# slp-rl/aero

Hardware: AMD Instinct MI355X
Metric: real-time-factor (audio-sec/wall-sec), Aero.forward STFT+U-Net+iSTFT, 4->16kHz nfft=512 hop=64 batch=64 per GPU (higher is better)
Workload: dtype f16; 1 GPU; batch=64 synthetic 2s white-noise clips per GPU, 4->16 kHz, aero_4-16_512_64 (nfft=512 hop=64), random-init weights seed 2036, inference, inputs resident in HBM; global_batch=64, clip_samples=8000, frames=501, parallelism=clips sharded over 1 GPU(s), no data-path collective, precision=fp16 operands/storage, fp32 accumulate; STFT/iSTFT/statistics fp32

## Files before the change

### aero_amd/_lib.py

```python
import ctypes as C
import os

_HERE = os.path.dirname(os.path.abspath(__file__))
DEFAULT_LIB = os.path.join(_HERE, 'libaero_hip.so')

ACT_NONE, ACT_RELU, ACT_GELU, ACT_GLU, ACT_SNAKE = 0, 1, 2, 3, 4

i32, i64, vp, fp, dp = C.c_int32, C.c_int64, C.c_void_p, C.c_void_p, C.c_void_p


class ConvDesc(C.Structure):
    _fields_ = [('src0', vp), ('s0_b', i64), ('s0_f', i64), ('s0_t', i64), ('C0', i32),
                ('src1', vp), ('s1_b', i64), ('s1_f', i64), ('s1_t', i64), ('C1', i32),
                ('weight', vp), ('bias', fp),
                ('dst', vp), ('d_b', i64), ('d_f', i64), ('d_t', i64),
                ('dst_f32', i32), ('dst_f_off', i32), ('dst_F', i32),
                ('B', i32), ('Fin', i32), ('Fout', i32), ('T', i32), ('M', i32),
                ('transposed', i32), ('fstride', i32),
                ('ntaps', i32), ('df', i32 * 9), ('dt', i32 * 9),
                ('act', i32),
                ('res', vp), ('r_b', i64), ('r_f', i64), ('r_t', i64),
                ('post_add', fp), ('batch_scale', fp), ('batch_shift', fp),
                ('stats', dp), ('stat_count', C.c_double),
                ('stat_mode', i32), ('stat_G', i32), ('stat_per_row', i32), ('stat_eps', C.c_float),
# ... 103 lines not shown

class SeanetConvDesc(C.Structure):
    _fields_ = [('x', vp), ('wimg', vp), ('bias', fp), ('add', vp), ('y', vp),
                ('B', i32), ('Tin', i32), ('Cin', i32), ('Tq', i32), ('M', i32), ('K', i32), ('stride', i32), ('dil', i32), ('pad', i32),
                ('reflect', i32), ('ksteps', i32), ('R', i32), ('P', i32), ('Tout', i32), ('Cout', i32), ('act', i32), ('in_slope', C.c_float)]


class SeanetResDesc(C.Structure):
    _fields_ = [('x', vp), ('w1', vp), ('w2s', vp), ('b1', fp), ('b2s', fp), ('add', vp), ('y', vp),
                ('B', i32), ('T', i32), ('C', i32), ('d', i32), ('ks1', i32), ('ks2', i32), ('slope', C.c_float)]


DCONV_MAX_DEPTH = 4


class DconvLayer(C.Structure):
    _fields_ = [('w1', vp), ('w2', vp), ('consts', fp), ('snake_a', fp),
                ('dilation', i32), ('norm1', i32), ('norm2', i32), ('reserved', i32)]


class DconvDesc(C.Structure):
    _fields_ = [('x', vp), ('y', vp), ('R', i32), ('T', i32), ('C', i32), ('hidden', i32), ('depth', i32), ('act', i32),
                ('F', i32), ('eps', C.c_float), ('layer', DconvLayer * DCONV_MAX_DEPTH)]


_PROTOS = {
    'aero_version': (C.c_char_p, []),
    'aero_last_error': (C.c_char_p, []),
    'aero_last_kernel_name': (C.c_char_p, []),
    'aero_stft_fwd': (i32, [fp, i32, i32, i32, i32, i32, fp, i32, fp, i32, dp, i32, vp]),
    'aero_stft_dft_table_bytes': (i64, [i32]),
    'aero_stft_dft_table': (i32, [fp, i32, i32, vp, vp]),
    'aero_stft_dft_fwd': (i32, [fp, i32, i32, i32, i32, i32, i32, vp, fp, i32, dp, i32, vp]),
    'aero_stft_dft_norm_fwd': (i32, [fp, i32, i32, i32, i32, i32, i32, vp, i32, dp, i32, vp, fp, vp]),
    'aero_spec_normalize': (i32, [fp, i32, i64, dp, vp, fp, vp]),
    'aero_istft_fwd': (i32, [fp, i32, i32, i32, i32, i32, fp, fp, fp, i32, vp]),
    'aero_istft_pitch': (i32, [i32, i32, i32, C.POINTER(i32), C.POINTER(i32)]),
    'aero_istft_pitched_fwd': (i32, [fp, i32, i32, i32, i32, i32, i32, i32, fp, fp, fp, i32, vp]),
    'aero_conv_fwd': (i32, [C.POINTER(ConvDesc), vp]),
    'aero_split_finish': (i32, [fp, i32, fp, i32, vp, i64, i32, vp]),
    'aero_adam_step': (i32, [fp, fp, fp, fp, i64, C.c_float, C.c_float, C.c_float, C.c_float, i32, C.c_float, vp]),
    'aero_adam_step_dev': (i32, [fp, fp, fp, fp, i64, C.c_float, C.c_float, C.c_float, C.c_float, fp, C.c_float, vp]),
    'aero_conv_wgrad': (i32, [C.POINTER(WgradDesc), vp]),
    'aero_conv_wgrad_chunks': (i32, [i32, i32, i32, i32, i32]),
    'aero_norm_bwd_reduce': (i32, [C.POINTER(NormBwdDesc), vp]),
    'aero_norm_bwd_apply': (i32, [C.POINTER(NormBwdDesc), vp]),
    'aero_istft_bwd_prep': (i32, [fp, fp, fp, i32, i32, i32, i32, i32, vp]),
    'aero_istft_bwd_pack': (i32, [fp, fp, i32, i32, i32, i32, i32, vp]),
    'aero_conv_tile_m': (i32, [i32]),
    'aero_conv_ring_bm': (i32, [i32, i32]),
    'aero_convtr_tail_finish': (i32, [fp, fp, fp, fp, fp, fp, i32, i32, i32, i32, i32, vp]),
    'aero_convtr_tail_finish_pitched': (i32, [fp, fp, fp, fp, fp, fp, i32, i32, i32, i32, i32, i32, i32, vp]),
    'aero_conv_kernel_name': (i32, [C.POINTER(ConvDesc), C.c_char_p, i32]),
    'aero_norm_stats': (i32, [C.POINTER(NormDesc), vp]),
    'aero_norm_apply': (i32, [C.POINTER(NormDesc), vp]),
    'aero_gram_stats': (i32, [C.POINTER(GramDesc), vp]),
    'aero_lstm_fwd': (i32, [C.POINTER(LstmDesc), vp]),
    'aero_lstm_geometry': (i32, [i32, C.POINTER(i32), C.POINTER(i32)]),
    'aero_lstm_geometry_in': (i32, [i32, i32, C.POINTER(i32)]),
    'aero_localstate_fwd': (i32, [C.POINTER(AttnDesc), vp]),
    'aero_freqfc_fwd': (i32, [C.POINTER(FreqFcDesc), vp]),
    'aero_ftb_first_fwd': (i32, [C.POINTER(FtbFirstDesc), vp]),
    'aero_enc0_fwd': (i32, [C.POINTER(Enc0Desc), vp]),
    'aero_dconv_row_fwd': (i32, [C.POINTER(DconvDesc), vp]),
    'aero_dconv_row_fits': (i32, [i32, i32, i32, i32]),
    'aero_lstm_bwd': (i32, [C.POINTER(LstmBwdDesc), vp]),
    'aero_lstm_bwd_k4p': (i32, [i32]),
    'aero_localstate_bwd': (i32, [C.POINTER(AttnBwdDesc), vp]),
    'aero_freqfc_wgrad': (i32, [vp, vp, vp, fp, fp, i32, i32, i32, i32, i32, vp]),
    'aero_ftb_gate_bwd': (i32, [vp, vp, vp, vp, vp, vp, i32, i32, i32, i32, vp]),
    'aero_sum_bt': (i32, [vp, fp, i32, i32, i32, i32, C.c_float, vp]),
    'aero_frames_op': (i32, [vp, vp, i32, i32, i32, i32, i32, i32, i32, vp]),
    'aero_stft_loss_sums': (i32, [fp, fp, i64, C.c_float, dp, i32, dp, vp]),
    'aero_stft_loss_bwd': (i32, [fp, fp, i64, C.c_float, dp, C.c_float, C.c_float, fp, fp, vp]),
    'aero_irfft_frames': (i32, [fp, i32, i32, i32, i32, fp, fp, vp]),
    'aero_stft_adj_fold': (i32, [fp, fp, i32, i32, i32, i32, i32, i32, vp]),
    'aero_add_f16': (i32, [vp, vp, vp, i64, C.c_float, vp]),
    'aero_scale_cast': (i32, [fp, i32, i64, fp, vp, C.c_float, vp, fp, vp]),
    'aero_scale_f32': (i32, [fp, i64, fp, vp]),
    'aero_gather_pack': (i32, [vp, vp, i32, vp, vp, i64, i32, vp]),
    'aero_debug_probe': (i32, [vp, i32, i32, i32, vp, vp]),
    'aero_bn_running_update': (i32, [dp, i32, C.c_double, C.c_float, fp, fp, vp, vp]),
    'aero_gconv1d_mfma_ok': (i32, [i32, i32, i32, i32, i32, i32, i32]),
    'aero_weightnorm_fwd': (i32, [fp, fp, fp, i32, i32, vp]),
    'aero_weightnorm_bwd': (i32, [fp, i64, i64, i64, fp, fp, fp, fp, fp, fp, fp, fp, i32, i32, i32, i32, vp]),
    'aero_gconv1d_wgrad_slabs': (i32, [i32, i32, i32, i32, i32, i32, i32, i32, i32]),
    'aero_rescale_f16': (i32, [vp, fp, vp, fp, i64, vp, C.c_float, vp, fp, vp]),
    'aero_gconv1d_fwd': (i32, [C.POINTER(GconvDesc), vp]),
# ... 87 lines not shown
```

### aero_amd/csrc/aero_hip.hip

```cpp
#include "aero_common.h"
#ifdef AERO_PART
#define AERO_IN(p) (AERO_PART == (p))
#else
#define AERO_IN(p) 1
#endif
#if AERO_IN(0)
#include "k_attn.h"
#include "k_lstm.h"
#include "k_norm.h"
#include "k_gram.h"
#include "k_optim.h"
#endif
#if AERO_IN(1)
#include "k_stft.h"
#include "k_train.h"
#endif
#if AERO_IN(2)
#include "k_conv.h"
#endif
#if AERO_IN(6)
#include "k_conv_ring.h"
#endif
#if AERO_IN(7)
#include "k_pw.h"
// ... 399 lines not shown
    name[0] = 0;
    int rc = aero_conv_launch(d, nullptr, &err, name);
    return rc == AERO_OK ? AERO_OK : aero_fail(rc, err);
}

int aero_split_finish(const float* acc, int32_t nsplit, const float* bias, int32_t act, void* dst, int64_t npos, int32_t M, void* stream) {
    const char* err = "";
    int rc = aero_split_finish_launch(acc, nsplit, bias, act, dst, npos, M, (hipStream_t)stream, &err);
    return aero_finish(rc, err);
}

#endif

#if AERO_IN(3)

int aero_freqfc_fwd(const aero_freqfc_desc* d, void* stream) {
    const char* err = "";
    int rc = aero_freqfc_launch(d, (hipStream_t)stream, &err);
    return aero_finish(rc, err);
}

int aero_dconv_row_fwd(const aero_dconv_desc* d, void* stream) {
    const char* err = "";
    int rc = aero_dconv_launch(d, (hipStream_t)stream, &err);
    return aero_finish(rc, err);
}

int aero_dconv_row_fits(int T, int C, int hidden, int max_dilation) { return aero_dconv_row_fits_impl(T, C, hidden, max_dilation); }

int aero_enc0_fwd(const aero_enc0_desc* d, void* stream) {
    const char* err = "";
    int rc = aero_enc0_launch(d, (hipStream_t)stream, &err);
    return aero_finish(rc, err);
}

int aero_ftb_first_fwd(const aero_ftb_first_desc* d, void* stream) {
    const char* err = "";
    int rc = aero_ftb_first_launch(d, (hipStream_t)stream, &err);
    return aero_finish(rc, err);
}

#endif

#if AERO_IN(4)

int aero_conv_wgrad(const aero_wgrad_desc* d, void* stream) {
    const char* err = "";
    int rc = aero_conv_wgrad_launch(d, (hipStream_t)stream, &err);
    return aero_finish(rc, err);
}

// ... 342 lines not shown
```

### aero_amd/csrc/k_dconv.h

```cpp
#pragma once
#include "aero_common.h"

struct AeroDconvK {
    aero_dconv_desc d;
    int HP;
    int logp;
    int T16;
    int PADR;
};

static inline int aero_dconv_logp(int C) {
    int s = (2 * C) & 255, g = 256;
    if (s) g = s & -s;
    int P = 256 / g, l = 0;
    while ((1 << l) < P) ++l;
    return l;
}

static inline size_t aero_dconv_lds_bytes(int T, int C, int hidden, int maxdil) {
    if (T < 1 || C < 8 || C % 8 || hidden < 4 || hidden % 4 || hidden > 32 || maxdil < 1 || maxdil > 64) return 0;
    const int HP = (hidden + 15) / 16 * 16, K1p = (3 * C + 31) / 32 * 32, T16 = (T + 15) / 16 * 16;
    const int padr = (maxdil + 7) / 8 * 8;
    const int xrows = T16 + 2 * padr, logp = aero_dconv_logp(C);
    const size_t xs = (size_t)xrows * C + (size_t)((xrows >> logp) + 1) * 8;
    const size_t w1 = (size_t)HP * K1p, w2 = (size_t)2 * C * HP;
    const size_t halves = (xs + w1 + w2 + 7) / 8 * 8;
    const size_t floats = 3 * HP + 3 * 2 * C + C + 2 * 16 * 2 + 8;
    return halves * 2 + floats * 4;
}

static __device__ __forceinline__ void aero_dconv_moments(float s1, float s2, float inv_n, float eps, float& mean, float& rstd) {
    const float m = s1 * inv_n;
    double var = (double)s2 * (double)inv_n - (double)m * (double)m;
    const float vf = fmaxf((float)var, 0.f) + eps;
    float r = aero_rsqrt(vf);
    r = r * (1.5f - 0.5f * vf * r * r);
    mean = m;
    rstd = r;
}

static inline int aero_dconv_nw(size_t lds_bytes, int T) { return (lds_bytes > 80 * 1024 || T > 512) ? 16 : 8; }

template <int HM, int NF2, int NW, int MAXF>
__global__ __launch_bounds__(NW * 64, 4) void aero_dconv_row_kernel(AeroDconvK p) {
    constexpr int C = NF2 * 8, HP = HM * 16, NK1 = (3 * C + 31) / 32, K1p = NK1 * 32, CU = NF2, NT = NW * 64;
    const aero_dconv_desc& d = p.d;
    const int T = d.T, hidden = d.hidden;
    const int xrows = p.T16 + 2 * p.PADR;
    h16* xs = (h16*)AERO_DYN_SMEM;
    h16* w1s = xs + xrows * C + ((xrows >> p.logp) + 1) * 8;
    h16* w2s = w1s + HP * K1p;
    float* c1 = (float*)(xs + ((int)(w2s + 2 * C * HP - xs) + 7) / 8 * 8);
    float* c2 = c1 + 3 * HP;
    float* sc = c2 + 3 * 2 * C;
    float* red = sc + C;
    const int tid = threadIdx.x, lane = tid & 63, wave = aero_uniform(tid >> 6);
    const int g = lane >> 4, col = lane & 15;
    const int row = aero_xcd_swizzle((int)blockIdx.x, (int)gridDim.x);
    const int nfrag = p.T16 >> 4;
    auto xoff = [&](int r) { return r * C + ((r >> p.logp) << 3); };

    {
        const h16* src = (const h16*)d.x + (int64_t)row * T * C;
        const int gsz = (CU << p.logp) + 1;
        const int total = xrows * CU + (xrows >> p.logp) + 1;
        for (int ub = wave * 64; ub < total; ub += NT) {
// ... 155 lines not shown
        for (int mf = 0; mf < NF2; ++mf) {
            const f32x4 A2 = *(const f32x4*)&c2[2 * C + mf * 16 + g * 4], B2 = *(const f32x4*)&c2[4 * C + mf * 16 + g * 4];
            const f32x2 ls = *(const f32x2*)&sc[mf * 8 + g * 2];
            h16x4 wf[HM];
#pragma unroll
            for (int ks = 0; ks < HM; ++ks) wf[ks] = *(const h16x4*)&w2s[(mf * HM + ks) * 256 + w2lane];
#pragma unroll
            for (int f = 0; f < MAXF; ++f) {
                if (wave + f * NW >= nfrag) continue;
                h16* xr = &xs[xlane[f] + mf * 8];
                const h16x2 xv = *(const h16x2*)xr;
                f32x4 v = (f32x4){0.f, 0.f, 0.f, 0.f};
#pragma unroll
                for (int ks = 0; ks < HM; ++ks) v = __builtin_amdgcn_mfma_f32_16x16x16f16(wf[ks], hB[f][ks], v, 0, 0, 0);
                v = v * A2 + B2;
                constexpr float NL2E = -1.4426950408889634f;
                const float g0 = aero_rcp(1.f + aero_exp2(v[1] * NL2E)), g1 = aero_rcp(1.f + aero_exp2(v[3] * NL2E));
                const float o0 = fmaf(v[0] * g0, ls[0], (float)xv[0]);
                const float o1 = fmaf(v[2] * g1, ls[1], (float)xv[1]);
                if (msk[f] != 0.f) *(h16x2*)xr = (h16x2){(h16)o0, (h16)o1};
            }
        }
    }
    __syncthreads();
    {
        h16* dst = (h16*)d.y + (int64_t)row * T * C;
        for (int u = tid; u < T * CU; u += NT) {
            const int t = u / CU, s = u - t * CU;
            *(h16x8*)(dst + (int64_t)t * C + s * 8) = *(const h16x8*)&xs[xoff(t + p.PADR) + s * 8];
        }
    }
}

static int aero_dconv_row_fits_impl(int T, int C, int hidden, int maxdil) {
    const size_t b = aero_dconv_lds_bytes(T, C, hidden, maxdil);
    const int nf2 = C / 8;
    const bool inst = nf2 == 2 || nf2 == 4 || nf2 == 6 || nf2 == 8 || nf2 == 12 || nf2 == 16;
    return b != 0 && b <= 160 * 1024 && inst && T <= (nf2 >= 12 && aero_dconv_nw(b, T) == 16 ? 512 : 1024);
}

static int aero_dconv_launch(const aero_dconv_desc* d, hipStream_t stream, const char** err) {
    if (!d || !d->x || !d->y) { *err = "dconv: null pointer"; return AERO_ERR_ARG; }
    if (d->R < 1 || d->T < 1 || d->depth < 1 || d->depth > AERO_DCONV_MAX_DEPTH || d->F < 1) { *err = "dconv: bad geometry"; return AERO_ERR_ARG; }
    if (d->act != AERO_ACT_RELU && d->act != AERO_ACT_GELU && d->act != AERO_ACT_SNAKE && d->act != AERO_ACT_NONE) { *err = "dconv: unsupported act"; return AERO_ERR_UNSUPPORTED; }
    int maxdil = 1;
    for (int l = 0; l < d->depth; ++l) {
        const aero_dconv_layer& L = d->layer[l];
        if (!L.w1 || !L.w2 || !L.consts) { *err = "dconv: null layer weights"; return AERO_ERR_ARG; }
        if (d->act == AERO_ACT_SNAKE && !L.snake_a) { *err = "dconv: snake needs a"; return AERO_ERR_ARG; }
        if (L.dilation < 1) { *err = "dconv: dilation"; return AERO_ERR_ARG; }
        if ((((uintptr_t)L.w1 | (uintptr_t)L.w2 | (uintptr_t)L.consts) & 15)) { *err = "dconv: unaligned weights"; return AERO_ERR_ARG; }
        maxdil = L.dilation > maxdil ? L.dilation : maxdil;
    }
    if ((((uintptr_t)d->x | (uintptr_t)d->y) & 15)) { *err = "dconv: unaligned rows"; return AERO_ERR_ARG; }
    if (!aero_dconv_row_fits_impl(d->T, d->C, d->hidden, maxdil)) { *err = "dconv: row does not fit the LDS (or C % 8, hidden % 4, hidden > 32)"; return AERO_ERR_UNSUPPORTED; }
    if (d->R > 0x7fffffff) { *err = "dconv: grid too large"; return AERO_ERR_ARG; }
    AeroDconvK p;
    p.d = *d;
    p.HP = (d->hidden + 15) / 16 * 16;
    p.logp = aero_dconv_logp(d->C);
    p.T16 = (d->T + 15) / 16 * 16;
    p.PADR = (maxdil + 7) / 8 * 8;
    const size_t lds = aero_dconv_lds_bytes(d->T, d->C, d->hidden, maxdil);
    const int nw = aero_dconv_nw(lds, d->T), nf2 = d->C / 8;
    dim3 grid((unsigned)d->R), block((unsigned)nw * 64);
#define AERO_DCONV_GO(NF2_)                                                                                            \
    do {                                                                                                               \
        constexpr int MF16 = NF2_ >= 12 ? 2 : 4;      \
        if (nw == 16 && (d->T + 15) / 16 > 16 * MF16) { *err = "dconv: row too long"; return AERO_ERR_UNSUPPORTED; }    \
        if (p.HP == 16 && nw == 8) AERO_LAUNCH_DYN((aero_dconv_row_kernel<1, NF2_, 8, 4>), grid, block, lds, stream, p);  \
        else if (p.HP == 16) AERO_LAUNCH_DYN((aero_dconv_row_kernel<1, NF2_, 16, MF16>), grid, block, lds, stream, p);       \
        else if (nw == 8) AERO_LAUNCH_DYN((aero_dconv_row_kernel<2, NF2_, 8, 4>), grid, block, lds, stream, p);           \
        else AERO_LAUNCH_DYN((aero_dconv_row_kernel<2, NF2_, 16, MF16>), grid, block, lds, stream, p);                       \
    } while (0)
    switch (nf2) {
        case 2: AERO_DCONV_GO(2); break;
        case 4: AERO_DCONV_GO(4); break;
        case 6: AERO_DCONV_GO(6); break;
        case 8: AERO_DCONV_GO(8); break;
        case 12: AERO_DCONV_GO(12); break;
        default: AERO_DCONV_GO(16); break;
    }
#undef AERO_DCONV_GO
    return AERO_OK;
}
```

### aero_amd/engine.py

```python
import ctypes as C
import math
import os

import torch

from . import _lib, pack
from ._lib import ACT_GELU, ACT_GLU, ACT_NONE, ACT_RELU, ACT_SNAKE


def _ptr(t):
    return None if t is None else t.data_ptr()


def _strides4(t):
    assert t.dim() == 4 and (t.shape[3] == 1 or t.stride(3) == 1), (t.shape, t.stride())
    return t.stride(0), t.stride(1), t.stride(2)


_SIDE_STREAMS = {}


def side_streams(device, n):
    dev = torch.device(device)
    if dev.type == 'cuda' and dev.index is None:
# ... 209 lines not shown
        if split_acc is not None:
            self._call('aero_split_finish', 'aero_split_finish_kernel', 0.0, split_acc.numel() * 4 + dst.numel() * 2, _ptr(split_acc), tap_split,
                       _ptr(spec.bias), act, _ptr(dst), B * Fout * T, spec.M, self.stream(dst))
        if tail is not None:
            return tail_lo, tail_hi
        return dst

    def convtr_tail_finish(self, lo, hi, bias, scale, shift, dst_F, pad, cin, pitched=None):
        B, Fin, T, _ = lo.shape
        self._shape_note = f'convtr tail finish F={Fin}->{dst_F}'
        if pitched is not None and pitched != (T, 0):
            pitch, toff = pitched
            dst = torch.empty(B, dst_F, pitch, 2, dtype=torch.float32, device=lo.device)
            self._call('aero_convtr_tail_finish_pitched', 'aero_convtr_tail_finish_kernel', 2.0 * B * Fin * T * 16 * cin, lo.numel() * 8 + B * dst_F * T * 8,
                       _ptr(lo), _ptr(hi), _ptr(bias), _ptr(scale), _ptr(shift), _ptr(dst), B, Fin, T, dst_F, pad, pitch, toff, self.stream(lo))
            dst._aero_pitched = (T, toff)
            return dst
        dst = torch.empty(B, dst_F, T, 2, dtype=torch.float32, device=lo.device)
        self._call('aero_convtr_tail_finish', 'aero_convtr_tail_finish_kernel', 2.0 * B * Fin * T * 16 * cin, lo.numel() * 8 + dst.numel() * 4,
                   _ptr(lo), _ptr(hi), _ptr(bias), _ptr(scale), _ptr(shift), _ptr(dst), B, Fin, T, dst_F, pad, self.stream(lo))
        return dst

    def pw(self, spec, x, B, F, T, res=None, post_add=None, stats=None, count=None, gamma=None, beta=None, layer_scale=None,
           eps=1e-5, tag='aero_pw_kernel', x1=None):
        Mout = spec.M // 2 if spec.act == ACT_GLU else spec.M
        dst = torch.empty(B, F, T, Mout, dtype=torch.float16, device=x.device)
        d = _lib.PwDesc()
        d.x = _ptr(x)
        d.x_b, d.x_f, d.x_t = _strides4(x)
        d.C = spec.C
        d.wimg, d.bias = _ptr(spec.wimg), _ptr(spec.bias)
        d.stats = _ptr(stats)
        d.stat_count = float(count) if stats is not None else 0.0
        d.stat_eps = eps
        d.gamma, d.beta, d.layer_scale, d.post_add = _ptr(gamma), _ptr(beta), _ptr(layer_scale), _ptr(post_add)
        d.res = _ptr(res)
        if res is not None:
            d.r_b, d.r_f, d.r_t = _strides4(res)
        d.dst = _ptr(dst)
        d.d_b, d.d_f, d.d_t = _strides4(dst)
        d.B, d.F, d.T, d.M, d.act = B, F, T, spec.M, spec.act
        if x1 is not None:
            d.x1 = _ptr(x1)
            d.x1_b, d.x1_f, d.x1_t = _strides4(x1)
            d.C0 = x.shape[-1]
        self._shape_note = f'pw M={spec.M} C={spec.C} F={F} act={spec.act} res={int(res is not None)} norm={int(stats is not None)}'
        nb = x.numel() // x.shape[-1] * (2 * spec.C + 2 * Mout * (2 if res is not None else 1))
# ... 151 lines not shown
Ops.ftb_first = _ftb_first


def _enc0(self, xn, u, g, P, conv, Fo, stride, pad, act):
    B, F, T, _ = xn.shape
    Cc, M = P['C'], conv.M
    out = torch.empty(B, Fo, T, M, dtype=torch.float16, device=xn.device)
    d = _lib.Enc0Desc()
    d.xn, d.u, d.g = _ptr(xn), _ptr(u), _ptr(g)
    d.rs, d.a_re, d.a_im, d.bias_f = _ptr(P['rs']), _ptr(P['a_re']), _ptr(P['a_im']), _ptr(P['bias'])
    d.wc, d.bias_c, d.dst = _ptr(conv.weight), _ptr(conv.bias), _ptr(out)
    d.B, d.F, d.T, d.C, d.M, d.Fo = B, F, T, Cc, M, Fo
    d.ktaps, d.stride, d.pad, d.act = len(conv.df), stride, pad, act
    flops = 2.0 * B * Fo * T * M * len(conv.df) * Cc
    self._shape_note = f'enc0 C={Cc} M={M} taps={len(conv.df)} F={F}->{Fo}'
    self._call('aero_enc0_fwd', 'aero_enc0_kernel', flops, B * F * T * 8 + B * Fo * T * M * 2 + g.numel() * 2,
               C.byref(d), self.stream(out))
    return out


Ops.enc0 = _enc0


def _dconv_row(self, x, layers, act, F, eps=1e-5):
    B, Fq, T, Cc = x.shape
    out = torch.empty_like(x)
    d = _lib.DconvDesc()
    d.x, d.y = _ptr(x), _ptr(out)
    d.R, d.T, d.C, d.hidden, d.depth, d.act, d.F, d.eps = B * Fq, T, Cc, layers[0]['hidden'], len(layers), act, F, eps
    flops = 0.0
    for i, L in enumerate(layers):
        l = d.layer[i]
        l.w1, l.w2, l.consts, l.snake_a = _ptr(L['w1']), _ptr(L['w2']), _ptr(L['consts']), _ptr(L.get('snake_a'))
        l.dilation, l.norm1, l.norm2 = L['dilation'], L['norm1'], L['norm2']
        flops += 2.0 * B * Fq * T * L['hidden'] * (3 * Cc + 2 * Cc)
    self._shape_note = f'dconv rows C={Cc} hidden={layers[0]["hidden"]} depth={len(layers)} F={Fq}'
    self._call('aero_dconv_row_fwd', 'aero_dconv_row_kernel', flops, 2 * x.numel() * 2, C.byref(d), self.stream(x))
    return out


def _dconv_row_fits(self, T, Cc, hidden, maxdil):
    return bool(self.lib.cdll.aero_dconv_row_fits(T, Cc, hidden, maxdil))


Ops.dconv_row = _dconv_row
Ops.dconv_row_fits = _dconv_row_fits


def blstm_frames(T, W=200, S=100):
    n = math.ceil(T / S)
    if n >= 3 and T <= (n - 1) * S + S // 2:
        n -= 1
    return n


def _hann_padded(win_length, n_fft, device):
    w = torch.zeros(n_fft, dtype=torch.float32)
    left = (n_fft - win_length) // 2
    w[left:left + win_length] = torch.hann_window(win_length, periodic=True, dtype=torch.float32)
    return w.to(device)


class _ShapeCache(dict):
    BOUNDED = ('hidpad', 'ones', 'env', 'graph')
    MAX_PER_KIND = 8
# ... 22 lines not shown
    _mark_base = None
    _out_pitch = None

    def __init__(self, model, lib=None):
        self.model = model
        self.lib = lib if lib is not None else _lib.load()
        self.ops = Ops(self.lib)
        self._key = None
        self._params, self._epoch = None, 0
        self._tables = _ShapeCache()
        self.streams = int(os.environ.get('AERO_STREAMS', '0'))
        self.stagger = int(os.environ.get('AERO_STAGGER', '0'))
        self.prof_streams = False
        self.use_graph = os.environ.get('AERO_GRAPH', '0') != '0'
        self.fuse_dconv_tail = os.environ.get('AERO_FUSE_DCONV', '1') != '0'
        self.gram_stats = os.environ.get('AERO_GRAM_STATS', '1') != '0'
        self.fuse_stats = {'0': False, '1': True}.get(os.environ.get('AERO_FUSE_STATS', 'auto'), 'auto')
        self.ring_stats = os.environ.get('AERO_RING_STATS', '1') != '0'
        self.fuse_lstm_proj = True
        self.collapse_first_ftb = True
        self.split_taps = os.environ.get('AERO_TAP_SPLIT', '1') != '0'
        self.use_pw = os.environ.get('AERO_PW', '1') != '0'
        self.fuse_dconv_row = os.environ.get('AERO_DCONV_ROW', '1') != '0'
        self.fuse_enc0 = os.environ.get('AERO_FUSE_ENC0', '1') != '0'
        self.fuse_tail = os.environ.get('AERO_FUSE_TAIL', '1') != '0'
        self.pitched_out = os.environ.get('AERO_PITCHED_OUT', '1') != '0'

    def _weights_key(self, device):
        if self._params is None:
            self._params = list(self.model.state_dict(keep_vars=True).values())
        return (str(device), self._epoch) + tuple((p.data_ptr(), p._version) for p in self._params)

    def invalidate(self):
        self._epoch += 1
        self._params = None

    def _prepare(self, device):
        key = self._weights_key(device)
        if key != self._key:
            self._params = None
            self._pack(device)
            self._key = key
            for k in [k for k in self._tables if isinstance(k, tuple) and k and k[0] == 'graph']:
                del self._tables[k]

    def _pack(self, device):
# ... 51 lines not shown
                    f32 = lambda t: t.float().to(device).contiguous()
                    wg = torch.cat([w2a * Wp[:, 0][None, :], w2a * Wp[:, 1][None, :], w2a * bp[None, :]], 0)
                    L['ftb0_g'] = mk(wg[None, :, None, :], None, Cc, 0, [0], [0], device)
                    L['ftb0'] = dict(C=Cc, w2a=img.to(device=device, dtype=torch.float16).contiguous(),
                                     p0=f32(Wp[:, 0]), p1=f32(Wp[:, 1]), pb=f32(bp), rs=f32(wfc.sum(1)),
                                     a_re=f32(A[:, 0]), a_im=f32(A[:, 1]), bias=f32(w2b @ bp + b2))
            w, df, dt = pack.conv2d_taps(sd[f'{p}.conv.weight'], enc.pad, 0)
            L['conv'] = mk(w, sd[f'{p}.conv.bias'], w.shape[-1], 0, df, dt, device, fstride=enc.stride,
                           act=ACT_NONE if enc.norm else ACT_GELU)
            if enc.norm:
                L['norm1'] = (sd[f'{p}.norm1.weight'].to(device), sd[f'{p}.norm1.bias'].to(device))
            if enc.dconv is not None:
                L['dconv'] = self._pack_dconv(sd, f'{p}.dconv', enc.dconv, device)
            if enc.rewrite is not None:
                w, df, dt = pack.conv2d_taps(sd[f'{p}.rewrite.weight'], enc.context, enc.context)
                L['rewrite'] = mk(w, sd[f'{p}.rewrite.bias'], w.shape[-1], 0, df, dt, device,
                                  act=ACT_NONE if enc.norm else ACT_GLU)
                if enc.norm:
                    L['norm2'] = (sd[f'{p}.norm2.weight'].to(device), sd[f'{p}.norm2.bias'].to(device))
                    if len(df) == 1 and w.shape[-1] <= 384:
                        L['rewrite_pw'] = pack.make_pw_spec(w[0, :, 0, :], sd[f'{p}.rewrite.bias'], ACT_NONE, self.lib, device)
                elif len(df) == 1:
                    L['rewrite_pw'] = pack.make_pw_spec(w[0, :, 0, :], sd[f'{p}.rewrite.bias'], ACT_GLU, self.lib, device)
            P[p] = L
        for j, dec in enumerate(m.decoder):
            p = f'decoder.{j}'
            L = {}
            half = dec.chin // 2
            if dec.rewrite is not None:
                w, df, dt = pack.conv2d_taps(sd[f'{p}.rewrite.weight'], dec.context, dec.context)
                L['rewrite'] = mk(w, sd[f'{p}.rewrite.bias'], half, half, df, dt, device,
                                  act=ACT_NONE if dec.norm else ACT_GLU)
                if dec.norm:
                    L['norm1'] = (sd[f'{p}.norm1.weight'].to(device), sd[f'{p}.norm1.bias'].to(device))
            w, df, dt = pack.convtr_taps(sd[f'{p}.conv_tr.weight'], dec.stride)
            act = ACT_NONE if (dec.norm or dec.last) else ACT_GELU
            L['conv_tr'] = mk(w, sd[f'{p}.conv_tr.bias'], w.shape[-1], 0, df, dt, device, transposed=1,
                              fstride=dec.stride, act=act)
            if dec.last and not dec.norm and dec.rewrite is not None:
                timg = pack.convtr_tail_image(sd[f'{p}.conv_tr.weight'], dec.stride, device)
                rw = L['rewrite']
                if (timg is not None and rw.M == 192 and rw.tiled_bm == 192 and len(rw.df) == 9 and timg.shape[1] == 96 and dec.pad == 2
                        and dec.kernel_size == 8):
                    L['tail'] = (timg, sd[f'{p}.conv_tr.bias'].detach().float().to(device).contiguous())
            if not dec.last and os.environ.get('AERO_CONVTR_STACK', '1') != '0':
                st = pack.convtr_stacked_spec(sd[f'{p}.conv_tr.weight'], sd[f'{p}.conv_tr.bias'], dec.stride, device, act=act)
# ... 145 lines not shown
                outs.append(self._forward_one(part, want_spec, want_lr_spec, defer_istft=True, stage_cb=stage_cb if self.stagger else None))
            prev_events = events
        for st in self._tables[key]:
            cur.wait_stream(st)
        ys = []
        for o in outs:
            spec_out, hop, win, T, Lout = o[0]
            spec_out.record_stream(cur)
            y = self.ops.istft(spec_out, self.model.nfft, hop, self._window(win, mix.device), self._inv_env(win, hop, T, mix.device), Lout)
            ys.append(y.view(spec_out.shape[0], 1, Lout))
        res = [torch.cat(ys, 0)]
        for k in (1, 2):
            parts = [o[k] for o in outs]
            if parts[0] is None:
                res.append(None)
                continue
            for t in parts:
                t.record_stream(cur)
            res.append(torch.cat(parts, 0))
        return tuple(res)

    def _forward_graph(self, mix, want_spec, want_lr_spec):
        key = ('graph', tuple(mix.shape), str(mix.device), want_spec, want_lr_spec,
               self.fuse_dconv_tail, self.fuse_stats, self.collapse_first_ftb, self.fuse_lstm_proj, self.fuse_enc0, self.fuse_dconv_row, self.split_taps)
        self._prepare(mix.device)
        ent = self._tables.get(key)
        if ent is None:
            static_in = mix.clone()
            for _ in range(2):
                self._forward_one(static_in, want_spec, want_lr_spec)
            torch.cuda.synchronize(mix.device)
            g = torch.cuda.CUDAGraph()
            with torch.cuda.graph(g):
                static_out = self._forward_one(static_in, want_spec, want_lr_spec)
            ent = self._tables[key] = (g, static_in, static_out)
        g, static_in, static_out = ent
        static_in.copy_(mix)
        g.replay()
        return tuple(None if t is None else t.clone() for t in static_out)

    def _forward_one(self, mix, want_spec=False, want_lr_spec=False, train=False, defer_istft=False, stage_cb=None):
        m, ops, P = self.model, self.ops, None
        self._train = train
        if stage_cb is None:
            stage_cb = self.stage_hook
        self._check_input(mix)
        if m.in_channels != 1 or m.out_channels != 1:
# ... 151 lines not shown
                del self._tables[k]
            self._tables[key] = R
        return self._tables[key]

    def _encode_tail(self, i, enc, L, x, B, Fq, T, y_pre=None):
        ops = self.ops
        Fo = (Fq + 2 * enc.pad - enc.kernel_size) // enc.stride + 1
        if y_pre is not None:
            return self._encode_rest(i, enc, L, y_pre, B, Fo, T)
        ops.tag = 'stack'
        if enc.norm:
            st = self._stats_for(L['conv'].M, enc.norm_groups, B, Fo, x.device, spec=L['conv'])
            y = ops.conv(L['conv'], x, None, B, Fq, Fo, T, stat=self._acc(st, enc.norm_groups))
            ops.tag = ''
            y = ops.norm_act(y, enc.norm_groups, False, L['norm1'][0], L['norm1'][1], ACT_GELU, stats=st)
        else:
            y = ops.conv(L['conv'], x, None, B, Fq, Fo, T)
        ops.tag = ''
        return self._encode_rest(i, enc, L, y, B, Fo, T)

    def _encode_rest(self, i, enc, L, y, B, Fo, T):
        ops = self.ops
        self._mark(i + 0.25)
        if 'dconv' in L:
            self._mark_base = i
            y = self._dconv(enc.dconv, L['dconv'], y, B, Fo, T)
            self._mark_base = None
            self._mark(i + 0.75)
        if 'rewrite' in L:
            emb = self.P.get('freq_emb') if i == 0 else None
            if enc.norm:
                if emb is not None:
                    raise NotImplementedError('GroupNorm on encoder 0 together with the frequency embedding')
                st = self._stats_for(L['rewrite'].M, enc.norm_groups, B, Fo, y.device, spec=L['rewrite'])
                ops.tag = 'stack'
                if st is None and self.use_pw and L.get('rewrite_pw') is not None and y.is_contiguous():
                    r = ops.pw(L['rewrite_pw'], y, B, Fo, T)
                else:
                    r = ops.conv(L['rewrite'], y, None, B, Fo, Fo, T, stat=self._acc(st, enc.norm_groups))
                ops.tag = ''
                y = ops.norm_act(r, enc.norm_groups, False, L['norm2'][0], L['norm2'][1], ACT_GLU, stats=st)
            else:
                ops.tag = 'stack'
                if self.use_pw and L.get('rewrite_pw') is not None and y.is_contiguous():
                    y = ops.pw(L['rewrite_pw'], y, B, Fo, T, post_add=emb)
                else:
                    y = ops.conv(L['rewrite'], y, None, B, Fo, Fo, T, post_add=emb)
                ops.tag = ''
        elif i == 0 and 'freq_emb' in self.P:
            raise NotImplementedError('frequency embedding without a rewrite conv')
        return y, Fo

    def _mark(self, stage):
        if self.stage_hook is not None and not getattr(self, '_train', False):
            self.stage_hook(stage)

    def _dconv(self, dc, layers, x, B, Fo, T):
        ops = self.ops
        act = {'snake': ACT_SNAKE, 'gelu': ACT_GELU}.get(dc.act_func, ACT_RELU)
        if (self.fuse_dconv_row and all('row' in L for L in layers) and len(layers) <= _lib.DCONV_MAX_DEPTH and x.is_contiguous()
                and ops.dconv_row_fits(T, layers[0]['row']['C'], layers[0]['row']['hidden'], max(L['row']['dilation'] for L in layers))):
            return ops.dconv_row(x, [dict(L['row'], snake_a=L.get('snake_a')) for L in layers], act, Fo)
        for li, L in enumerate(layers):
            if li == 1 and getattr(self, '_mark_base', None) is not None:
                self._mark(self._mark_base + 0.5)
            g1 = L['gn1']
            st1 = None
            if g1 is not None and self._want_stats(L['conv1']) and L['conv1'].M > 16 and L['conv1'].M % 8 == 0:
                st1 = ops.new_stats(B, Fo, 1, True, x.device)
                h = ops.conv(L['conv1'], x, None, B, Fo, Fo, T, stat=dict(mode=1, stats=st1, G=1, per_row=True))
            else:
                h = ops.conv(L['conv1'], x, None, B, Fo, Fo, T)
            g2 = L['gn2']
            hp = L.get('hid_pad') if (g2 is not None and self.fuse_dconv_tail and L['conv2_glu'].M % 16 == 0) else None
# ... 159 lines not shown
```

### aero_amd/pack.py

```python
import math
from dataclasses import dataclass, field
from typing import List, Optional

import torch

from . import _lib


@dataclass
class ConvSpec:
    weight: torch.Tensor
    bias: Optional[torch.Tensor]
    M: int
    C0: int
    C1: int
    df: List[int]
    dt: List[int]
    transposed: int = 0
    fstride: int = 1
    act: int = _lib.ACT_NONE
    extra: dict = field(default_factory=dict)
    weight_tiled: Optional[torch.Tensor] = None
    tiled_bm: int = 0

# ... 213 lines not shown

def dconv_row_layer(w1, b1, g1, be1, w2, b2, g2, be2, scale, dilation, device):
    hid, Cc = w1.shape[0], w1.shape[1]
    HP, K1p = _round_up(hid, 16), _round_up(3 * Cc, 32)
    i1 = torch.zeros(HP, K1p)
    i1[:hid, :3 * Cc] = w1.detach().float().permute(0, 2, 1).reshape(hid, 3 * Cc)
    i2 = torch.zeros(2 * Cc, HP)
    i2[:, :hid] = glu_interleave(w2.detach().float())
    i2 = i2.reshape(2 * Cc // 16, 16, HP // 16, 4, 4).permute(0, 2, 3, 1, 4).contiguous()
    c = torch.zeros(3 * HP + 7 * Cc)
    c[:hid] = b1.detach().float()
    c[HP:HP + hid] = 1.0 if g1 is None else g1.detach().float()
    if be1 is not None:
        c[2 * HP:2 * HP + hid] = be1.detach().float()
    o = 3 * HP
    c[o:o + 2 * Cc] = glu_interleave(b2.detach().float())
    c[o + 2 * Cc:o + 4 * Cc] = 1.0 if g2 is None else glu_interleave(g2.detach().float())
    if be2 is not None:
        c[o + 4 * Cc:o + 6 * Cc] = glu_interleave(be2.detach().float())
    c[o + 6 * Cc:] = 1.0 if scale is None else scale.detach().float()
    return dict(w1=i1.to(device=device, dtype=torch.float16).contiguous(), w2=i2.to(device=device, dtype=torch.float16).contiguous(),
                consts=c.to(device).contiguous(), norm1=int(g1 is not None), norm2=int(g2 is not None), dilation=int(dilation),
                C=Cc, hidden=hid)
```

### include/aero_hip.h

```cpp
#ifndef AERO_HIP_H
#define AERO_HIP_H
#include <stdint.h>

#ifdef __cplusplus
extern "C" {
#endif

#define AERO_OK 0
#define AERO_ERR_ARG (-1)
#define AERO_ERR_LAUNCH (-2)
#define AERO_ERR_UNSUPPORTED (-3)

enum { AERO_ACT_NONE = 0, AERO_ACT_RELU = 1, AERO_ACT_GELU = 2, AERO_ACT_GLU = 3, AERO_ACT_SNAKE = 4 };

const char* aero_version(void);
const char* aero_last_error(void);
const char* aero_last_kernel_name(void);

int aero_stft_fwd(const float* x, int32_t nsig, int32_t L, int32_t Lp, int32_t n_fft, int32_t hop,
                  const float* window, int32_t n_bins, float* spec, int32_t T, double* stats,
                  int32_t sig_per_item, void* stream);

int64_t aero_stft_dft_table_bytes(int32_t n_fft);
int aero_stft_dft_table(const float* window, int32_t n_fft, int32_t win_off, void* table, void* stream);
// ... 120 lines not shown
typedef struct {
    const void* xn; const void* u; const void* g;
    const float* rs; const float* a_re; const float* a_im; const float* bias_f;
    const void* wc; const float* bias_c;
    void* dst;
    int32_t B, F, T, C, M, Fo, ktaps, stride, pad, act;
} aero_enc0_desc;
int aero_enc0_fwd(const aero_enc0_desc* d, void* stream);

#define AERO_DCONV_MAX_DEPTH 4
typedef struct {
    const void* w1; const void* w2; const float* consts; const float* snake_a;
    int32_t dilation, norm1, norm2, reserved;
} aero_dconv_layer;
typedef struct {
    const void* x; void* y;
    int32_t R, T, C, hidden, depth, act, F;
    float eps;
    aero_dconv_layer layer[AERO_DCONV_MAX_DEPTH];
} aero_dconv_desc;
int aero_dconv_row_fwd(const aero_dconv_desc* d, void* stream);
int aero_dconv_row_fits(int T, int C, int hidden, int max_dilation);

int aero_adam_step(float* p, const float* g, float* m, float* v, int64_t n, float lr, float beta1, float beta2, float eps,
                   int32_t step, float grad_scale, void* stream);
int aero_adam_step_dev(float* p, const float* g, float* m, float* v, int64_t n, float lr, float beta1, float beta2, float eps,
                       const float* bc, float grad_scale, void* stream);


typedef struct {
    const void* dy; int64_t dy_b, dy_f, dy_t;
    const void* x; int64_t x_b, x_f, x_t;
    float* dw; float* db;
    int32_t B, Fin, Fout, T, M, C, ntaps, fstride;
    int32_t df[9], dt[9];
    float* slabs; int32_t nslab;
    int32_t store, dw_layout, dw_rowlen, dw_coff;
} aero_wgrad_desc;
int aero_conv_wgrad(const aero_wgrad_desc* d, void* stream);
int aero_conv_wgrad_chunks(int32_t M, int32_t C, int32_t ntaps, int32_t nrows, int32_t T);

typedef struct {
    const void* x; int64_t x_b, x_f, x_t;
    const void* dy; int64_t dy_b, dy_f, dy_t;
    void* dx; int64_t dx_b, dx_f, dx_t;
    int32_t B, F, T, C, G, per_row;
// ... 144 lines not shown
```

Measured before the change: 15280 audio-sec/wall-sec.

## Fuse encoder rewrite 1x1 GLU conv into the per-row dconv kernel tail

Adds a templated RW tail to the row-resident dconv kernel. After the residual dconv layers finish in LDS, it loads the rewrite 1x1 conv weights, bias and an optional frequency-embedding add, then applies the GLU conv with MFMA in place before writing the final output with arbitrary strides. This removes a separate pointwise-conv launch and the HBM round trip of the dconv output in encoder layers. The cost is higher LDS use, which can lower occupancy or make some shapes fall back to the unfused path.

Result: faster. 15470 audio-sec/wall-sec, median of 6 (+1.3%).

```diff
diff --git a/aero_amd/_lib.py b/aero_amd/_lib.py
--- a/aero_amd/_lib.py
+++ b/aero_amd/_lib.py
@@ -149,6 +149,11 @@
 class DconvDesc(C.Structure):
     _fields_ = [('x', vp), ('y', vp), ('R', i32), ('T', i32), ('C', i32), ('hidden', i32), ('depth', i32), ('act', i32),
                 ('F', i32), ('eps', C.c_float), ('layer', DconvLayer * DCONV_MAX_DEPTH)]
+
+
+class DconvRewriteDesc(C.Structure):
+    _fields_ = [('dconv', DconvDesc), ('rw_w', vp), ('rw_bias', fp), ('post_add', fp),
+                ('dst', vp), ('d_b', i64), ('d_f', i64), ('d_t', i64)]
 
 
 _PROTOS = {
@@ -191,6 +196,8 @@
     'aero_enc0_fwd': (i32, [C.POINTER(Enc0Desc), vp]),
     'aero_dconv_row_fwd': (i32, [C.POINTER(DconvDesc), vp]),
     'aero_dconv_row_fits': (i32, [i32, i32, i32, i32]),
+    'aero_dconv_row_rewrite_fwd': (i32, [C.POINTER(DconvRewriteDesc), vp]),
+    'aero_dconv_row_rewrite_fits': (i32, [i32, i32, i32, i32]),
     'aero_lstm_bwd': (i32, [C.POINTER(LstmBwdDesc), vp]),
     'aero_lstm_bwd_k4p': (i32, [i32]),
     'aero_localstate_bwd': (i32, [C.POINTER(AttnBwdDesc), vp]),
diff --git a/aero_amd/csrc/aero_hip.hip b/aero_amd/csrc/aero_hip.hip
--- a/aero_amd/csrc/aero_hip.hip
+++ b/aero_amd/csrc/aero_hip.hip
@@ -445,11 +445,20 @@
 
 int aero_dconv_row_fwd(const aero_dconv_desc* d, void* stream) {
     const char* err = "";
-    int rc = aero_dconv_launch(d, (hipStream_t)stream, &err);
+    int rc = aero_dconv_launch(d, nullptr, (hipStream_t)stream, &err);
     return aero_finish(rc, err);
 }
 
 int aero_dconv_row_fits(int T, int C, int hidden, int max_dilation) { return aero_dconv_row_fits_impl(T, C, hidden, max_dilation); }
+
+int aero_dconv_row_rewrite_fwd(const aero_dconv_rewrite_desc* d, void* stream) {
+    const char* err = "";
+    if (!d) return aero_fail(AERO_ERR_ARG, "dconv rewrite: null descriptor");
+    int rc = aero_dconv_launch(&d->dconv, d, (hipStream_t)stream, &err);
+    return aero_finish(rc, err);
+}
+
+int aero_dconv_row_rewrite_fits(int T, int C, int hidden, int max_dilation) { return aero_dconv_row_fits_impl(T, C, hidden, max_dilation, true); }
 
 int aero_enc0_fwd(const aero_enc0_desc* d, void* stream) {
     const char* err = "";
diff --git a/aero_amd/csrc/k_dconv.h b/aero_amd/csrc/k_dconv.h
--- a/aero_amd/csrc/k_dconv.h
+++ b/aero_amd/csrc/k_dconv.h
@@ -7,6 +7,10 @@
     int logp;
     int T16;
     int PADR;
+    const void* rw_w;
+    const float* rw_b;
+    const float* rw_add;
+    void* out; int64_t o_b, o_f, o_t;
 };
 
 static inline int aero_dconv_logp(int C) {
@@ -29,6 +33,15 @@
     return halves * 2 + floats * 4;
 }
 
+static inline size_t aero_dconv_rw_lds_bytes(int T, int C, int hidden, int maxdil) {
+    const size_t base = aero_dconv_lds_bytes(T, C, hidden, maxdil);
+    if (!base || C % 16) return 0;
+    const int T16 = (T + 15) / 16 * 16, padr = (maxdil + 7) / 8 * 8, xrows = T16 + 2 * padr;
+    const size_t xbytes = ((size_t)xrows * C + (size_t)((xrows >> aero_dconv_logp(C)) + 1) * 8) * 2;
+    const size_t tail = (size_t)2 * C * ((C + 31) / 32 * 32) * 2 + (size_t)3 * C * 4;
+    return xbytes + (base - xbytes > tail ? base - xbytes : tail);
+}
+
 static __device__ __forceinline__ void aero_dconv_moments(float s1, float s2, float inv_n, float eps, float& mean, float& rstd) {
     const float m = s1 * inv_n;
     double var = (double)s2 * (double)inv_n - (double)m * (double)m;
@@ -41,7 +54,7 @@
 
 static inline int aero_dconv_nw(size_t lds_bytes, int T) { return (lds_bytes > 80 * 1024 || T > 512) ? 16 : 8; }
 
-template <int HM, int NF2, int NW, int MAXF>
+template <int HM, int NF2, int NW, int MAXF, bool RW = false>
 __global__ __launch_bounds__(NW * 64, 4) void aero_dconv_row_kernel(AeroDconvK p) {
     constexpr int C = NF2 * 8, HP = HM * 16, NK1 = (3 * C + 31) / 32, K1p = NK1 * 32, CU = NF2, NT = NW * 64;
     const aero_dconv_desc& d = p.d;
@@ -243,25 +256,70 @@
             }
         }
     }
+    if constexpr (RW) {
+        constexpr int NKR = (C + 31) / 32, KR = NKR * 32;
+        h16* wr = w1s;
+        float* rb = (float*)(wr + 2 * C * KR);
+        float* re = rb + 2 * C;
+        __syncthreads();
+        for (int ub = wave * 64; ub < 2 * C * KR / 8; ub += NT)
+            if (ub + lane < 2 * C * KR / 8) aero_glds16((const h16*)p.rw_w + (ub + lane) * 8, wr + ub * 8);
+        for (int ub = wave * 64; ub < 2 * C / 4; ub += NT)
+            if (ub + lane < 2 * C / 4) aero_glds16((const h16*)(p.rw_b + (ub + lane) * 4), (h16*)rb + ub * 8);
+        for (int ub = wave * 64; ub < C / 4; ub += NT)
+            if (ub + lane < C / 4) aero_glds16(p.rw_add ? (const h16*)(p.rw_add + (int64_t)(row % d.F) * C + (ub + lane) * 4) : aero_zero_page, (h16*)re + ub * 8);
+        __syncthreads();
+        h16x8 xb[MAXF][NKR];
+        int xrow[MAXF];
+#pragma unroll
+        for (int f = 0; f < MAXF; ++f) {
+            const int cf = wave + f * NW;
+            xrow[f] = xoff((cf < nfrag ? cf : 0) * 16 + col + p.PADR);
+#pragma unroll
+            for (int ks = 0; ks < NKR; ++ks) {
+                xb[f][ks] = (h16x8){0, 0, 0, 0, 0, 0, 0, 0};
+                if (ks * 32 + 24 < C || ks * 32 + g * 8 < C) xb[f][ks] = *(const h16x8*)&xs[xrow[f] + ks * 32 + g * 8];
+            }
+        }
+#pragma unroll
+        for (int mf = 0; mf < NF2; ++mf) {
+            const f32x4 bias = *(const f32x4*)&rb[mf * 16 + g * 4];
+            const f32x2 pe = *(const f32x2*)&re[mf * 8 + g * 2];
+            h16x8 wa[NKR];
+#pragma unroll
+            for (int ks = 0; ks < NKR; ++ks) wa[ks] = *(const h16x8*)&wr[(mf * NKR + ks) * 512 + lane * 8];
+#pragma unroll
+            for (int f = 0; f < MAXF; ++f) {
+                if (wave + f * NW >= nfrag) continue;
+                f32x4 v = bias;
+#pragma unroll
+                for (int ks = 0; ks < NKR; ++ks) v = __builtin_amdgcn_mfma_f32_16x16x32_f16(wa[ks], xb[f][ks], v, 0, 0, 0);
+                constexpr float NL2E = -1.4426950408889634f;
+                const float g0 = aero_rcp(1.f + aero_exp2(v[1] * NL2E)), g1 = aero_rcp(1.f + aero_exp2(v[3] * NL2E));
+                *(h16x2*)&xs[xrow[f] + mf * 8 + g * 2] = (h16x2){(h16)fmaf(v[0], g0, pe[0]), (h16)fmaf(v[2], g1, pe[1])};
+            }
+        }
+    }
     __syncthreads();
     {
-        h16* dst = (h16*)d.y + (int64_t)row * T * C;
+        h16* dst = RW ? (h16*)p.out + (int64_t)(row / d.F) * p.o_b + (int64_t)(row % d.F) * p.o_f : (h16*)d.y + (int64_t)row * T * C;
+        const int64_t dt = RW ? p.o_t : (int64_t)C;
         for (int u = tid; u < T * CU; u += NT) {
             const int t = u / CU, s = u - t * CU;
-            *(h16x8*)(dst + (int64_t)t * C + s * 8) = *(const h16x8*)&xs[xoff(t + p.PADR) + s * 8];
-        }
-    }
-}
-
-static int aero_dconv_row_fits_impl(int T, int C, int hidden, int maxdil) {
-    const size_t b = aero_dconv_lds_bytes(T, C, hidden, maxdil);
+            *(h16x8*)(dst + (int64_t)t * dt + s * 8) = *(const h16x8*)&xs[xoff(t + p.PADR) + s * 8];
+        }
+    }
+}
+
+static int aero_dconv_row_fits_impl(int T, int C, int hidden, int maxdil, bool rw = false) {
+    const size_t b = rw ? aero_dconv_rw_lds_bytes(T, C, hidden, maxdil) : aero_dconv_lds_bytes(T, C, hidden, maxdil);
     const int nf2 = C / 8;
     const bool inst = nf2 == 2 || nf2 == 4 || nf2 == 6 || nf2 == 8 || nf2 == 12 || nf2 == 16;
     return b != 0 && b <= 160 * 1024 && inst && T <= (nf2 >= 12 && aero_dconv_nw(b, T) == 16 ? 512 : 1024);
 }
 
-static int aero_dconv_launch(const aero_dconv_desc* d, hipStream_t stream, const char** err) {
-    if (!d || !d->x || !d->y) { *err = "dconv: null pointer"; return AERO_ERR_ARG; }
+static int aero_dconv_launch(const aero_dconv_desc* d, const aero_dconv_rewrite_desc* rw, hipStream_t stream, const char** err) {
+    if (!d || !d->x || (!rw && !d->y)) { *err = "dconv: null pointer"; return AERO_ERR_ARG; }
     if (d->R < 1 || d->T < 1 || d->depth < 1 || d->depth > AERO_DCONV_MAX_DEPTH || d->F < 1) { *err = "dconv: bad geometry"; return AERO_ERR_ARG; }
     if (d->act != AERO_ACT_RELU && d->act != AERO_ACT_GELU && d->act != AERO_ACT_SNAKE && d->act != AERO_ACT_NONE) { *err = "dconv: unsupported act"; return AERO_ERR_UNSUPPORTED; }
     int maxdil = 1;
@@ -273,8 +331,14 @@
         if ((((uintptr_t)L.w1 | (uintptr_t)L.w2 | (uintptr_t)L.consts) & 15)) { *err = "dconv: unaligned weights"; return AERO_ERR_ARG; }
         maxdil = L.dilation > maxdil ? L.dilation : maxdil;
     }
-    if ((((uintptr_t)d->x | (uintptr_t)d->y) & 15)) { *err = "dconv: unaligned rows"; return AERO_ERR_ARG; }
-    if (!aero_dconv_row_fits_impl(d->T, d->C, d->hidden, maxdil)) { *err = "dconv: row does not fit the LDS (or C % 8, hidden % 4, hidden > 32)"; return AERO_ERR_UNSUPPORTED; }
+    if ((((uintptr_t)d->x | (rw ? 0 : (uintptr_t)d->y)) & 15)) { *err = "dconv: unaligned rows"; return AERO_ERR_ARG; }
+    if (rw) {
+        if (!rw->rw_w || !rw->rw_bias || !rw->dst) { *err = "dconv rewrite: null pointer"; return AERO_ERR_ARG; }
+        if ((((uintptr_t)rw->rw_w | (uintptr_t)rw->rw_bias | (uintptr_t)rw->post_add | (uintptr_t)rw->dst) & 15) || ((rw->d_b | rw->d_f | rw->d_t) & 7) || rw->d_t < d->C)
+            { *err = "dconv rewrite: unaligned weights / output rows"; return AERO_ERR_ARG; }
+        if (d->R % d->F) { *err = "dconv rewrite: R is not a multiple of F"; return AERO_ERR_ARG; }
+    }
+    if (!aero_dconv_row_fits_impl(d->T, d->C, d->hidden, maxdil, rw != nullptr)) { *err = "dconv: row does not fit the LDS (or C % 8, hidden % 4, hidden > 32; with the rewrite tail C % 16)"; return AERO_ERR_UNSUPPORTED; }
     if (d->R > 0x7fffffff) { *err = "dconv: grid too large"; return AERO_ERR_ARG; }
     AeroDconvK p;
     p.d = *d;
@@ -282,17 +346,27 @@
     p.logp = aero_dconv_logp(d->C);
     p.T16 = (d->T + 15) / 16 * 16;
     p.PADR = (maxdil + 7) / 8 * 8;
-    const size_t lds = aero_dconv_lds_bytes(d->T, d->C, d->hidden, maxdil);
+    p.rw_w = rw ? rw->rw_w : nullptr;
+    p.rw_b = rw ? rw->rw_bias : nullptr;
+    p.rw_add = rw ? rw->post_add : nullptr;
+    p.out = rw ? rw->dst : nullptr;
+    p.o_b = rw ? rw->d_b : 0; p.o_f = rw ? rw->d_f : 0; p.o_t = rw ? rw->d_t : 0;
+    const size_t lds = rw ? aero_dconv_rw_lds_bytes(d->T, d->C, d->hidden, maxdil) : aero_dconv_lds_bytes(d->T, d->C, d->hidden, maxdil);
     const int nw = aero_dconv_nw(lds, d->T), nf2 = d->C / 8;
     dim3 grid((unsigned)d->R), block((unsigned)nw * 64);
-#define AERO_DCONV_GO(NF2_)                                                                                            \
+#define AERO_DCONV_GO2(NF2_, RW_)                                                                                      \
     do {                                                                                                               \
         constexpr int MF16 = NF2_ >= 12 ? 2 : 4;      \
         if (nw == 16 && (d->T + 15) / 16 > 16 * MF16) { *err = "dconv: row too long"; return AERO_ERR_UNSUPPORTED; }    \
-        if (p.HP == 16 && nw == 8) AERO_LAUNCH_DYN((aero_dconv_row_kernel<1, NF2_, 8, 4>), grid, block, lds, stream, p);  \
-        else if (p.HP == 16) AERO_LAUNCH_DYN((aero_dconv_row_kernel<1, NF2_, 16, MF16>), grid, block, lds, stream, p);       \
-        else if (nw == 8) AERO_LAUNCH_DYN((aero_dconv_row_kernel<2, NF2_, 8, 4>), grid, block, lds, stream, p);           \
-        else AERO_LAUNCH_DYN((aero_dconv_row_kernel<2, NF2_, 16, MF16>), grid, block, lds, stream, p);                       \
+        if (p.HP == 16 && nw == 8) AERO_LAUNCH_DYN((aero_dconv_row_kernel<1, NF2_, 8, 4, RW_>), grid, block, lds, stream, p);  \
+        else if (p.HP == 16) AERO_LAUNCH_DYN((aero_dconv_row_kernel<1, NF2_, 16, MF16, RW_>), grid, block, lds, stream, p);       \
+        else if (nw == 8) AERO_LAUNCH_DYN((aero_dconv_row_kernel<2, NF2_, 8, 4, RW_>), grid, block, lds, stream, p);           \
+        else AERO_LAUNCH_DYN((aero_dconv_row_kernel<2, NF2_, 16, MF16, RW_>), grid, block, lds, stream, p);                       \
+    } while (0)
+#define AERO_DCONV_GO(NF2_)                                                                                            \
+    do {                                                                                                               \
+        if (rw) AERO_DCONV_GO2(NF2_, true);                                                                            \
+        else AERO_DCONV_GO2(NF2_, false);                                                                              \
     } while (0)
     switch (nf2) {
         case 2: AERO_DCONV_GO(2); break;
@@ -303,5 +377,6 @@
         default: AERO_DCONV_GO(16); break;
     }
 #undef AERO_DCONV_GO
+#undef AERO_DCONV_GO2
     return AERO_OK;
 }
diff --git a/aero_amd/engine.py b/aero_amd/engine.py
--- a/aero_amd/engine.py
+++ b/aero_amd/engine.py
@@ -255,7 +255,10 @@
         return dst
 
     def pw(self, spec, x, B, F, T, res=None, post_add=None, stats=None, count=None, gamma=None, beta=None, layer_scale=None,
-           eps=1e-5, tag='aero_pw_kernel', x1=None):
+           eps=1e-5, tag='aero_pw_kernel', x1=None, dconv=None):
+        if dconv is not None:
+            assert spec.act == ACT_GLU and res is None and stats is None and layer_scale is None and x1 is None
+            return self.dconv_row(x, dconv['layers'], dconv['act'], F, rewrite=dconv['rw'], post_add=post_add)
         Mout = spec.M // 2 if spec.act == ACT_GLU else spec.M
         dst = torch.empty(B, F, T, Mout, dtype=torch.float16, device=x.device)
         d = _lib.PwDesc()
@@ -453,11 +456,12 @@
 Ops.enc0 = _enc0
 
 
-def _dconv_row(self, x, layers, act, F, eps=1e-5):
+def _dconv_row(self, x, layers, act, F, eps=1e-5, rewrite=None, post_add=None):
     B, Fq, T, Cc = x.shape
     out = torch.empty_like(x)
-    d = _lib.DconvDesc()
-    d.x, d.y = _ptr(x), _ptr(out)
+    r = _lib.DconvRewriteDesc()
+    d = r.dconv
+    d.x, d.y = _ptr(x), (None if rewrite is not None else _ptr(out))
     d.R, d.T, d.C, d.hidden, d.depth, d.act, d.F, d.eps = B * Fq, T, Cc, layers[0]['hidden'], len(layers), act, F, eps
     flops = 0.0
     for i, L in enumerate(layers):
@@ -465,13 +469,20 @@
         l.w1, l.w2, l.consts, l.snake_a = _ptr(L['w1']), _ptr(L['w2']), _ptr(L['consts']), _ptr(L.get('snake_a'))
         l.dilation, l.norm1, l.norm2 = L['dilation'], L['norm1'], L['norm2']
         flops += 2.0 * B * Fq * T * L['hidden'] * (3 * Cc + 2 * Cc)
-    self._shape_note = f'dconv rows C={Cc} hidden={layers[0]["hidden"]} depth={len(layers)} F={Fq}'
-    self._call('aero_dconv_row_fwd', 'aero_dconv_row_kernel', flops, 2 * x.numel() * 2, C.byref(d), self.stream(x))
+    if rewrite is None:
+        self._shape_note = f'dconv rows C={Cc} hidden={layers[0]["hidden"]} depth={len(layers)} F={Fq}'
+        self._call('aero_dconv_row_fwd', 'aero_dconv_row_kernel', flops, 2 * x.numel() * 2, C.byref(d), self.stream(x))
+        return out
+    r.rw_w, r.rw_bias, r.post_add, r.dst = _ptr(rewrite['w']), _ptr(rewrite['bias']), _ptr(post_add), _ptr(out)
+    r.d_b, r.d_f, r.d_t = _strides4(out)
+    self._shape_note = f'dconv rows + rewrite C={Cc} hidden={layers[0]["hidden"]} depth={len(layers)} F={Fq}'
+    self._call('aero_dconv_row_rewrite_fwd', 'aero_dconv_row_kernel', flops + 2.0 * B * Fq * T * 2 * Cc * Cc, 2 * x.numel() * 2, C.byref(r), self.stream(x))
     return out
 
 
-def _dconv_row_fits(self, T, Cc, hidden, maxdil):
-    return bool(self.lib.cdll.aero_dconv_row_fits(T, Cc, hidden, maxdil))
+def _dconv_row_fits(self, T, Cc, hidden, maxdil, rewrite=False):
+    fn = self.lib.cdll.aero_dconv_row_rewrite_fits if rewrite else self.lib.cdll.aero_dconv_row_fits
+    return bool(fn(T, Cc, hidden, maxdil))
 
 
 Ops.dconv_row = _dconv_row
@@ -540,6 +551,7 @@
         self.split_taps = os.environ.get('AERO_TAP_SPLIT', '1') != '0'
         self.use_pw = os.environ.get('AERO_PW', '1') != '0'
         self.fuse_dconv_row = os.environ.get('AERO_DCONV_ROW', '1') != '0'
+        self.fuse_dconv_rewrite = os.environ.get('AERO_DCONV_ROW_REWRITE', '1') != '0'
         self.fuse_enc0 = os.environ.get('AERO_FUSE_ENC0', '1') != '0'
         self.fuse_tail = os.environ.get('AERO_FUSE_TAIL', '1') != '0'
         self.pitched_out = os.environ.get('AERO_PITCHED_OUT', '1') != '0'
@@ -637,6 +649,8 @@
                         L['rewrite_pw'] = pack.make_pw_spec(w[0, :, 0, :], sd[f'{p}.rewrite.bias'], ACT_NONE, self.lib, device)
                 elif len(df) == 1:
                     L['rewrite_pw'] = pack.make_pw_spec(w[0, :, 0, :], sd[f'{p}.rewrite.bias'], ACT_GLU, self.lib, device)
+                    if L['rewrite_pw'] is not None and w.shape[1] == 2 * w.shape[-1]:
+                        L['rewrite_row'] = pack.dconv_rewrite_image(w[0, :, 0, :], sd[f'{p}.rewrite.bias'], device)
             P[p] = L
         for j, dec in enumerate(m.decoder):
             p = f'decoder.{j}'
@@ -828,7 +842,8 @@
 
     def _forward_graph(self, mix, want_spec, want_lr_spec):
         key = ('graph', tuple(mix.shape), str(mix.device), want_spec, want_lr_spec,
-               self.fuse_dconv_tail, self.fuse_stats, self.collapse_first_ftb, self.fuse_lstm_proj, self.fuse_enc0, self.fuse_dconv_row, self.split_taps)
+               self.fuse_dconv_tail, self.fuse_stats, self.collapse_first_ftb, self.fuse_lstm_proj, self.fuse_enc0, self.fuse_dconv_row, self.fuse_dconv_rewrite,
+               self.split_taps)
         self._prepare(mix.device)
         ent = self._tables.get(key)
         if ent is None:
@@ -1026,6 +1041,13 @@
     def _encode_rest(self, i, enc, L, y, B, Fo, T):
         ops = self.ops
         self._mark(i + 0.25)
+        if 'dconv' in L and self._row_rewrite_applies(enc, L, y, T):
+            layers = L['dconv']
+            act = {'snake': ACT_SNAKE, 'gelu': ACT_GELU}.get(enc.dconv.act_func, ACT_RELU)
+            y = ops.pw(L['rewrite_pw'], y, B, Fo, T, post_add=self.P.get('freq_emb') if i == 0 else None,
+                       dconv=dict(layers=[dict(Lr['row'], snake_a=Lr.get('snake_a')) for Lr in layers], act=act, rw=L['rewrite_row']))
+            self._mark(i + 0.75)
+            return y, Fo
         if 'dconv' in L:
             self._mark_base = i
             y = self._dconv(enc.dconv, L['dconv'], y, B, Fo, T)
@@ -1054,6 +1076,18 @@
         elif i == 0 and 'freq_emb' in self.P:
             raise NotImplementedError('frequency embedding without a rewrite conv')
         return y, Fo
+
+    def _row_rewrite_applies(self, enc, L, y, T):
+        layers = L['dconv']
+        if not (getattr(self, 'fuse_dconv_rewrite', False) and self.fuse_dconv_row and self.use_pw and not enc.norm
+                and not getattr(self, '_train', False) and L.get('rewrite_row') is not None and y.is_contiguous()
+                and all('row' in Lr for Lr in layers) and len(layers) <= _lib.DCONV_MAX_DEPTH):
+            return False
+        r0 = layers[0]['row']
+        if L['rewrite_row']['C'] != r0['C']:
+            return False
+        maxdil = max(Lr['row']['dilation'] for Lr in layers)
+        return self.ops.dconv_row_fits(T, r0['C'], r0['hidden'], maxdil) and self.ops.dconv_row_fits(T, r0['C'], r0['hidden'], maxdil, rewrite=True)
 
     def _mark(self, stage):
         if self.stage_hook is not None and not getattr(self, '_train', False):
diff --git a/aero_amd/pack.py b/aero_amd/pack.py
--- a/aero_amd/pack.py
+++ b/aero_amd/pack.py
@@ -259,3 +259,15 @@
     return dict(w1=i1.to(device=device, dtype=torch.float16).contiguous(), w2=i2.to(device=device, dtype=torch.float16).contiguous(),
                 consts=c.to(device).contiguous(), norm1=int(g1 is not None), norm2=int(g2 is not None), dilation=int(dilation),
                 C=Cc, hidden=hid)
+
+
+def dconv_rewrite_image(w, bias, device):
+    M, Cc = w.shape
+    if M != 2 * Cc or Cc % 16:
+        return None
+    ks = (Cc + 31) // 32
+    wi = torch.zeros(M, ks * 32)
+    wi[:, :Cc] = glu_interleave(w.detach().float().cpu())
+    img = wi.reshape(M // 16, 16, ks, 4, 8).permute(0, 2, 3, 1, 4).contiguous()
+    b = torch.zeros(M) if bias is None else glu_interleave(bias.detach().float().cpu())
+    return dict(w=img.to(device=device, dtype=torch.float16).contiguous(), bias=b.to(device).contiguous(), C=Cc)
diff --git a/include/aero_hip.h b/include/aero_hip.h
--- a/include/aero_hip.h
+++ b/include/aero_hip.h
@@ -166,6 +166,14 @@
 int aero_dconv_row_fwd(const aero_dconv_desc* d, void* stream);
 int aero_dconv_row_fits(int T, int C, int hidden, int max_dilation);
 
+typedef struct {
+    aero_dconv_desc dconv;
+    const void* rw_w; const float* rw_bias; const float* post_add;
+    void* dst; int64_t d_b, d_f, d_t;
+} aero_dconv_rewrite_desc;
+int aero_dconv_row_rewrite_fwd(const aero_dconv_rewrite_desc* d, void* stream);
+int aero_dconv_row_rewrite_fits(int T, int C, int hidden, int max_dilation);
+
 int aero_adam_step(float* p, const float* g, float* m, float* v, int64_t n, float lr, float beta1, float beta2, float eps,
                    int32_t step, float grad_scale, void* stream);
 int aero_adam_step_dev(float* p, const float* g, float* m, float* v, int64_t n, float lr, float beta1, float beta2, float eps,
```
